# WoojuLee24/OA-DG

Measured on AMD Instinct MI355X. Metric: images/sec training, Faster R-CNN R50-FPN + OA-DG, 1024x2048, higher is better.
Workload: dtype bf16

## Files before the change

oa-dg_amd/csrc/assign.hip:

```cpp
#include <cstring>
#include "common.h"
#include "../../include/oadg_hip.h"

namespace {

constexpr int AS_THREADS = 256;
constexpr int AS_MAXG = 1024;

struct AssignArgs {
    const float* boxes;
    long box_stride;
    const unsigned char* valid;
    const float* gts;
    const int* gt_counts;
    const int64_t* gt_labels;
    int B, N, Gmax;
    float pos_thr, neg_lo, neg_hi, min_pos;
    int match_low_quality;
    unsigned* gt_max;
    int64_t* gt_inds;
    float* max_overlaps;
    int64_t* labels;
    int* counts;
    long out_stride;
};

__device__ __forceinline__ unsigned fkey(float f) {
    const unsigned u = __float_as_uint(f);
    return (u & 0x80000000u) ? ~u : (u | 0x80000000u);
}
__device__ __forceinline__ float funkey(unsigned k) {
    return __uint_as_float((k & 0x80000000u) ? (k & 0x7fffffffu) : ~k);
}

__device__ __forceinline__ float iou_of(const float4 g, const float ga, const float4 b, const float ba) {
    const float ltx = fmaxf(g.x, b.x), lty = fmaxf(g.y, b.y);
    const float rbx = fminf(g.z, b.z), rby = fminf(g.w, b.w);
    const float w = fmaxf(rbx - ltx, 0.f), h = fmaxf(rby - lty, 0.f);
    const float overlap = w * h;
    float uni = (ga + ba) - overlap;
    uni = fmaxf(uni, 1e-6f);
    return overlap / uni;
}

__global__ __launch_bounds__(AS_THREADS) void assign_gtmax_kernel(AssignArgs a) {
    __shared__ float4 sg[AS_MAXG];
    __shared__ float sga[AS_MAXG];
    __shared__ unsigned smax[AS_MAXG];
    const int b = blockIdx.y;
    const int G = a.gt_counts[b];
    for (int g = threadIdx.x; g < G; g += AS_THREADS) {
        const float4 v = reinterpret_cast<const float4*>(a.gts)[(long)b * a.Gmax + g];
        sg[g] = v;
        sga[g] = (v.z - v.x) * (v.w - v.y);
        smax[g] = fkey(-1.f);
    }
    __syncthreads();
    const float* boxes = a.boxes + (long)b * a.box_stride;
    const int lane = threadIdx.x & 63;
    const long chunk = (long)gridDim.x * AS_THREADS;
    for (long base = (long)blockIdx.x * AS_THREADS; base < a.N; base += chunk) {
        const long n = base + threadIdx.x;
        const bool ok = n < a.N && (!a.valid || a.valid[(long)b * a.N + n]);
        float4 bx = make_float4(0.f, 0.f, 0.f, 0.f);
        if (n < a.N) bx = reinterpret_cast<const float4*>(boxes)[n];
        const float ba = (bx.z - bx.x) * (bx.w - bx.y);
        for (int g = 0; g < G; ++g) {
            float v = ok ? iou_of(sg[g], sga[g], bx, ba) : -1.f;
            v = wave_max(v);
            if (lane == 0) atomicMax(&smax[g], fkey(v));
        }
    }
    __syncthreads();
    for (int g = threadIdx.x; g < G; g += AS_THREADS) atomicMax(&a.gt_max[(long)b * a.Gmax + g], smax[g]);
}

__global__ __launch_bounds__(AS_THREADS) void assign_kernel(AssignArgs a) {
    __shared__ float4 sg[AS_MAXG];
    __shared__ float sga[AS_MAXG];
    __shared__ float sgm[AS_MAXG];
    __shared__ int red[2][AS_THREADS / 64];
    const int b = blockIdx.y;
    const int G = a.gt_counts[b];
    for (int g = threadIdx.x; g < G; g += AS_THREADS) {
        const float4 v = reinterpret_cast<const float4*>(a.gts)[(long)b * a.Gmax + g];
        sg[g] = v;
        sga[g] = (v.z - v.x) * (v.w - v.y);
        sgm[g] = funkey(a.gt_max[(long)b * a.Gmax + g]);
    }
    __syncthreads();
    const float* boxes = a.boxes + (long)b * a.box_stride;
    int npos = 0, nneg = 0;
    const long chunk = (long)gridDim.x * AS_THREADS;
    for (long n = (long)blockIdx.x * AS_THREADS + threadIdx.x; n < a.N; n += chunk) {
        const bool ok = !a.valid || a.valid[(long)b * a.N + n];
        const float4 bx = reinterpret_cast<const float4*>(boxes)[n];
        const float ba = (bx.z - bx.x) * (bx.w - bx.y);
        int64_t ind = -1;
        float mo = 0.f;
        if (G == 0) {
            ind = 0;
        } else {
            float best = -2.f;
            int arg = 0, last = 0;
            for (int g = 0; g < G; ++g) {
                const float v = ok ? iou_of(sg[g], sga[g], bx, ba) : -1.f;
                if (v > best) { best = v; arg = g; }
                if (a.match_low_quality && sgm[g] >= a.min_pos && v == sgm[g]) last = g + 1;
            }
            mo = best;
            if (best >= a.neg_lo && best < a.neg_hi) ind = 0;
            if (best >= a.pos_thr) ind = arg + 1;
            if (last > 0) ind = last;
        }
        if (!ok) ind = -1;
        a.gt_inds[(long)b * a.out_stride + n] = ind;
        a.max_overlaps[(long)b * a.out_stride + n] = mo;
        if (a.labels) a.labels[(long)b * a.out_stride + n] = ind > 0 ? a.gt_labels[(long)b * a.Gmax + (ind - 1)] : -1;
        npos += ind > 0;
        nneg += ind == 0;
    }
    npos = wave_sum_i(npos);
    nneg = wave_sum_i(nneg);
    const int lane = threadIdx.x & 63, w = threadIdx.x >> 6;
    if (lane == 0) { red[0][w] = npos; red[1][w] = nneg; }
    __syncthreads();
    if (threadIdx.x == 0) {
        int p = 0, q = 0;
        for (int i = 0; i < AS_THREADS / 64; ++i) { p += red[0][i]; q += red[1][i]; }
        if (p) atomicAdd(&a.counts[b * 2], p);
        if (q) atomicAdd(&a.counts[b * 2 + 1], q);
    }
}

__global__ void assign_init_kernel(unsigned* gt_max, int n, int* counts, int m) {
    const int i = blockIdx.x * blockDim.x + threadIdx.x;
    if (i < n) gt_max[i] = fkey(-1.f);
    if (i < m) counts[i] = 0;
}

struct RoiPrepArgs {
    oadg_roi_assign_image img[OADG_ROI_ASSIGN_MAX_IMAGES];
    int B, N, Gmax;
    float* boxes_full;
    int64_t* gt_inds_full;
    int64_t* labels_full;
    float* max_ov_full;
    unsigned char* valid;
    float* gts_pad;
    int64_t* gl_pad;
    int* gt_counts;
    unsigned* gt_max;
    int* counts;
};

__global__ __launch_bounds__(256) void roi_assign_prep_kernel(const RoiPrepArgs a) {
    const int b = blockIdx.y;
    const float* props = nullptr; const float* gts = nullptr; const int64_t* gl = nullptr;
    int stride = 4, G = 0;
#pragma unroll
    for (int i = 0; i < OADG_ROI_ASSIGN_MAX_IMAGES; ++i)
        if (i == b) { props = a.img[i].proposals; gts = a.img[i].gt_bboxes; gl = a.img[i].gt_labels;
                      stride = a.img[i].stride; G = a.img[i].num_gts; }
    const int rows = a.Gmax + a.N;
    const int r = blockIdx.x * 256 + threadIdx.x;
    if (r == 0) {
        a.gt_counts[b] = G;
        a.counts[2 * b] = 0; a.counts[2 * b + 1] = 0;
        if (a.Gmax == 0) a.gt_max[b] = fkey(-1.f);
    }
    if (r >= rows) return;
    const long o = (long)b * rows + r;
    if (r < a.Gmax) {
        float4 g = make_float4(0.f, 0.f, 0.f, 0.f);
        int64_t l = 0;
        if (r < G) { g = reinterpret_cast<const float4*>(gts)[r]; l = gl[r]; }
        reinterpret_cast<float4*>(a.gts_pad)[(long)b * a.Gmax + r] = g;
        a.gl_pad[(long)b * a.Gmax + r] = l;
        a.gt_max[(long)b * a.Gmax + r] = fkey(-1.f);
        const int j = r - (a.Gmax - G);
        if (j >= 0) {
            reinterpret_cast<float4*>(a.boxes_full)[o] = reinterpret_cast<const float4*>(gts)[j];
            a.gt_inds_full[o] = j + 1;
            a.labels_full[o] = gl[j];
            a.max_ov_full[o] = 1.0f;
        }
        return;
    }
    const int n = r - a.Gmax;
    const float* p = props + (long)n * stride;
    reinterpret_cast<float4*>(a.boxes_full)[o] = make_float4(p[0], p[1], p[2], p[3]);
    a.valid[(long)b * a.N + n] = stride >= 5 ? (p[4] >= 0.f ? 1 : 0) : 1;
}

}

extern "C" size_t oadg_max_iou_assign_workspace_bytes(int B, int Gmax) {
    return B > 0 && Gmax >= 0 ? (size_t)B * (Gmax > 0 ? Gmax : 1) * sizeof(unsigned) : 0;
}

extern "C" int oadg_max_iou_assign(const float* boxes, long box_stride, const unsigned char* valid, const float* gts,
                                   const int* gt_counts, const int64_t* gt_labels, int B, int N, int Gmax,
                                   float pos_iou_thr, float neg_iou_lo, float neg_iou_hi, float min_pos_iou,
                                   int match_low_quality, void* workspace, size_t workspace_bytes, int64_t* gt_inds,
                                   float* max_overlaps, int64_t* labels, int* counts, void* stream) {
    if (!boxes || !gt_counts || !gt_inds || !max_overlaps || !counts || !workspace) return OADG_EARG;
    if (B < 1 || N < 0 || Gmax < 0 || Gmax > AS_MAXG || (Gmax > 0 && !gts) || (labels && !gt_labels)) return OADG_EARG;
    if (workspace_bytes < oadg_max_iou_assign_workspace_bytes(B, Gmax)) return OADG_ESIZE;
    AssignArgs a;
    a.boxes = boxes; a.box_stride = box_stride; a.valid = valid; a.gts = gts; a.gt_counts = gt_counts;
    a.gt_labels = gt_labels; a.B = B; a.N = N; a.Gmax = Gmax;
    a.pos_thr = pos_iou_thr; a.neg_lo = neg_iou_lo; a.neg_hi = neg_iou_hi; a.min_pos = min_pos_iou;
    a.match_low_quality = match_low_quality;
    a.gt_max = (unsigned*)workspace; a.gt_inds = gt_inds; a.max_overlaps = max_overlaps; a.labels = labels;
    a.counts = counts; a.out_stride = N;
    hipStream_t st = (hipStream_t)stream;
    const int ninit = B * (Gmax > 0 ? Gmax : 1) > 2 * B ? B * (Gmax > 0 ? Gmax : 1) : 2 * B;
    hipLaunchKernelGGL(assign_init_kernel, dim3((ninit + 255) / 256), dim3(256), 0, st, a.gt_max,
                       B * (Gmax > 0 ? Gmax : 1), counts, 2 * B);
    OADG_LAUNCH_CHECK();
    if (N == 0) return OADG_OK;
    int bx = (N + AS_THREADS - 1) / AS_THREADS;
    if (bx > 256) bx = 256;
    if (Gmax > 0) {
        hipLaunchKernelGGL(assign_gtmax_kernel, dim3(bx, B), dim3(AS_THREADS), 0, st, a);
        OADG_LAUNCH_CHECK();
    }
    hipLaunchKernelGGL(assign_kernel, dim3(bx, B), dim3(AS_THREADS), 0, st, a);
    OADG_LAUNCH_CHECK();
    return OADG_OK;
}

extern "C" int oadg_roi_assign_add_gt(const oadg_roi_assign_image* images_host, int B, int N, int Gmax, float pos_iou_thr,
                                      float neg_iou_lo, float neg_iou_hi, float min_pos_iou, int match_low_quality,
                                      float* boxes_full, int64_t* gt_inds_full, int64_t* labels_full, float* max_ov_full,
                                      unsigned char* valid, float* gts_pad, int64_t* gl_pad, int* gt_counts,
                                      void* workspace, size_t workspace_bytes, int* counts, void* stream) {
    if (!images_host || B < 1 || B > OADG_ROI_ASSIGN_MAX_IMAGES || N < 1 || Gmax < 0 || Gmax > AS_MAXG || !boxes_full ||
        !gt_inds_full || !labels_full || !max_ov_full || !valid || !gt_counts || !workspace || !counts ||
        (Gmax > 0 && (!gts_pad || !gl_pad)))
        return OADG_EARG;
    if (workspace_bytes < oadg_max_iou_assign_workspace_bytes(B, Gmax)) return OADG_ESIZE;
    RoiPrepArgs p;
    std::memset(&p, 0, sizeof(p));
    for (int i = 0; i < B; ++i) {
        const oadg_roi_assign_image& im = images_host[i];
        if (!im.proposals || im.stride < 4 || im.num_gts < 0 || im.num_gts > Gmax ||
            (im.num_gts > 0 && (!im.gt_bboxes || !im.gt_labels)))
            return OADG_EARG;
        p.img[i] = im;
    }
    p.B = B; p.N = N; p.Gmax = Gmax; p.boxes_full = boxes_full; p.gt_inds_full = gt_inds_full;
    p.labels_full = labels_full; p.max_ov_full = max_ov_full; p.valid = valid; p.gts_pad = gts_pad; p.gl_pad = gl_pad;
    p.gt_counts = gt_counts; p.gt_max = (unsigned*)workspace; p.counts = counts;
    hipStream_t st = (hipStream_t)stream;
    const int rows = Gmax + N;
    hipLaunchKernelGGL(roi_assign_prep_kernel, dim3((rows + 255) / 256, B), dim3(256), 0, st, p);
    OADG_LAUNCH_CHECK();
    AssignArgs a;
    a.boxes = boxes_full + (size_t)Gmax * 4; a.box_stride = (long)rows * 4; a.valid = valid; a.gts = gts_pad;
    a.gt_counts = gt_counts; a.gt_labels = gl_pad; a.B = B; a.N = N; a.Gmax = Gmax;
    a.pos_thr = pos_iou_thr; a.neg_lo = neg_iou_lo; a.neg_hi = neg_iou_hi; a.min_pos = min_pos_iou;
    a.match_low_quality = match_low_quality; a.gt_max = (unsigned*)workspace;
    a.gt_inds = gt_inds_full + Gmax; a.max_overlaps = max_ov_full + Gmax; a.labels = labels_full + Gmax;
    a.counts = counts; a.out_stride = rows;
    int bx = (N + AS_THREADS - 1) / AS_THREADS;
    if (bx > 256) bx = 256;
    if (Gmax > 0) {
        hipLaunchKernelGGL(assign_gtmax_kernel, dim3(bx, B), dim3(AS_THREADS), 0, st, a);
        OADG_LAUNCH_CHECK();
    }
    hipLaunchKernelGGL(assign_kernel, dim3(bx, B), dim3(AS_THREADS), 0, st, a);
    OADG_LAUNCH_CHECK();
    return OADG_OK;
}
```

oa-dg_amd/csrc/nms.hip:

```cpp
#include "common.h"
#include <type_traits>

namespace {

constexpr int MAX_WORDS_PER_LANE = 8;

__device__ __forceinline__ float iou_f32(const float4 a, const float4 b) {
    const float left = fmaxf(a.x, b.x), right = fminf(a.z, b.z);
    const float top = fmaxf(a.y, b.y), bottom = fminf(a.w, b.w);
    const float w = fmaxf(right - left, 0.f), h = fmaxf(bottom - top, 0.f);
    const float inter = w * h;
    const float sa = (a.z - a.x) * (a.w - a.y);
    const float sb = (b.z - b.x) * (b.w - b.y);
    return inter / (sa + sb - inter);
}

__global__ __launch_bounds__(64) void nms_mask_kernel(const float4* __restrict__ boxes,
                                                      const int* __restrict__ counts, int Mmax,
                                                      int words, float thr,
                                                      unsigned long long* __restrict__ mask) {
    const int img = blockIdx.z, rb = blockIdx.y, cb = blockIdx.x;
    if (cb < rb) return;
    const int M = min(counts[img], Mmax);
    if (rb * 64 >= M || cb * 64 >= M) return;
    __shared__ float4 colbox[64];
    const float4* b = boxes + (size_t)img * Mmax;
    const int t = threadIdx.x;
    const int cidx = cb * 64 + t;
    colbox[t] = cidx < M ? b[cidx] : make_float4(0.f, 0.f, 0.f, 0.f);
    __syncthreads();
    const int r = rb * 64 + t;
    if (r >= M) return;
    const float4 me = b[r];
    unsigned long long bits = 0ull;
    const int ncol = min(64, M - cb * 64);
    const int start = (rb == cb) ? t + 1 : 0;
    for (int j = start; j < ncol; ++j)
        if (iou_f32(me, colbox[j]) > thr) bits |= 1ull << j;
    mask[((size_t)img * Mmax + r) * words + cb] = bits;
}

__device__ __forceinline__ unsigned wave_or32(unsigned v) {
    v |= (unsigned)__builtin_amdgcn_update_dpp(0, (int)v, 0x128, 0xf, 0xf, false);
    v |= (unsigned)__builtin_amdgcn_update_dpp(0, (int)v, 0x124, 0xf, 0xf, false);
    v |= (unsigned)__builtin_amdgcn_update_dpp(0, (int)v, 0x122, 0xf, 0xf, false);
    v |= (unsigned)__builtin_amdgcn_update_dpp(0, (int)v, 0x121, 0xf, 0xf, false);
    return (unsigned)__builtin_amdgcn_readlane((int)v, 0) | (unsigned)__builtin_amdgcn_readlane((int)v, 16) |
           (unsigned)__builtin_amdgcn_readlane((int)v, 32) | (unsigned)__builtin_amdgcn_readlane((int)v, 48);
}
__device__ __forceinline__ unsigned long long wave_or64(unsigned long long v) {
    return ((unsigned long long)wave_or32((unsigned)(v >> 32)) << 32) | wave_or32((unsigned)v);
}

template <int SLOTS, int ROUNDS>
__global__ __launch_bounds__(64) void nms_scan_kernel(const unsigned long long* __restrict__ mask,
                                                      const int* __restrict__ counts, int Mmax,
                                                      int words, int max_keep, int* __restrict__ keep,
                                                      int* __restrict__ keep_cnt) {
    const int img = blockIdx.x, lane = threadIdx.x;
    const int M = min(counts[img], Mmax);
    const unsigned long long* mk = mask + (size_t)img * Mmax * words;
    int* out = keep + (size_t)img * Mmax;
    unsigned long long removed[SLOTS];
    unsigned long long pend[2][ROUNDS * 8][SLOTS];
#pragma unroll
    for (int s = 0; s < SLOTS; ++s) {
        removed[s] = 0ull;
#pragma unroll
        for (int u = 0; u < ROUNDS * 8; ++u) pend[0][u][s] = pend[1][u][s] = 0ull;
    }
    int nkeep = 0, pend_rounds[2] = {0, 0};
    const int nchunks = (M + 63) / 64;
    auto row_words = [&](int c, unsigned long long& d, unsigned long long& n1, unsigned long long& n2) {
        const int row = c * 64 + lane;
        const bool ok = c < nchunks && row < M;
        const unsigned long long* r = mk + (size_t)(ok ? row : 0) * words;
        d = ok ? r[c] : 0ull;
        n1 = (ok && c + 1 < nchunks) ? r[c + 1] : 0ull;
        n2 = (ok && c + 2 < nchunks) ? r[c + 2] : 0ull;
    };
    auto merge = [&](int w, unsigned long long v) {
#pragma unroll
        for (int s = 0; s < SLOTS; ++s)
            if (s == (w >> 6) && lane == (w & 63)) removed[s] |= v;
    };
    unsigned long long diag, near1, near2;
    row_words(0, diag, near1, near2);
    auto chunk = [&](int cw, auto set_c) {
        constexpr int SET = decltype(set_c)::value;
        unsigned long long mine = 0ull;
#pragma unroll
        for (int s = 0; s < SLOTS; ++s)
            if (s == (cw >> 6)) mine = removed[s];
        const unsigned lo = (unsigned)__builtin_amdgcn_readlane((int)(unsigned)mine, cw & 63);
        const unsigned hi = (unsigned)__builtin_amdgcn_readlane((int)(unsigned)(mine >> 32), cw & 63);
        unsigned long long cur = ((unsigned long long)hi << 32) | lo;
        unsigned long long ndiag, nnear1, nnear2;
        row_words(cw + 1, ndiag, nnear1, nnear2);
        const int nb = min(64, M - cw * 64);
        const int myrow = cw * 64 + lane;
        unsigned long long avail = ~cur & (nb == 64 ? ~0ull : ((1ull << nb) - 1ull));
        unsigned long long kept = 0ull;
        int nk = nkeep;
        while (avail && nk < max_keep) {
            const int bit = __ffsll((long long)avail) - 1;
            kept |= 1ull << bit;
            ++nk;
            const unsigned dlo = __builtin_amdgcn_readlane((int)(unsigned)diag, bit);
            const unsigned dhi = __builtin_amdgcn_readlane((int)(unsigned)(diag >> 32), bit);
            const unsigned long long d = ((unsigned long long)dhi << 32) | dlo;
            avail &= ~d & ~((2ull << bit) - 1ull);
        }
        const bool me_kept = (kept >> lane) & 1ull;
        if (me_kept) out[nkeep + __popcll(kept & ((1ull << lane) - 1ull))] = myrow;
        nkeep = nk;
        merge(cw + 1, wave_or64(me_kept ? near1 : 0ull));
        merge(cw + 2, wave_or64(me_kept ? near2 : 0ull));
#pragma unroll
        for (int rd = 0; rd < ROUNDS; ++rd)
            if (rd < pend_rounds[SET]) {
#pragma unroll
                for (int s = 0; s < SLOTS; ++s)
#pragma unroll
                    for (int u = 0; u < 8; ++u) removed[s] |= pend[SET][rd * 8 + u][s];
            }
        unsigned long long todo = kept;
        auto far_round = [&](int* bits) {
#pragma unroll
            for (int u = 0; u < 8; ++u) {
                bits[u] = todo ? __ffsll((long long)todo) - 1 : -1;
                todo &= todo - 1ull;
            }
        };
        pend_rounds[SET] = 0;
#pragma unroll
        for (int rd = 0; rd < ROUNDS; ++rd) {
            if (!todo) break;
            ++pend_rounds[SET];
            int bits[8];
            far_round(bits);
#pragma unroll
            for (int s = 0; s < SLOTS; ++s) {
                const int w = lane + 64 * s;
                const bool far = w > cw + 2 && w < nchunks;
#pragma unroll
                for (int u = 0; u < 8; ++u)
                    pend[SET][rd * 8 + u][s] = (far && bits[u] >= 0) ? mk[(size_t)(cw * 64 + bits[u]) * words + w] : 0ull;
            }
        }
        while (todo) {
            int bits[8];
            far_round(bits);
#pragma unroll
            for (int s = 0; s < SLOTS; ++s) {
                const int w = lane + 64 * s;
                const bool far = w > cw + 2 && w < nchunks;
                unsigned long long v[8];
#pragma unroll
                for (int u = 0; u < 8; ++u)
                    v[u] = (far && bits[u] >= 0) ? mk[(size_t)(cw * 64 + bits[u]) * words + w] : 0ull;
#pragma unroll
                for (int u = 0; u < 8; ++u) removed[s] |= v[u];
            }
        }
        diag = ndiag; near1 = nnear1; near2 = nnear2;
    };
    for (int cw = 0; cw < nchunks && nkeep < max_keep; cw += 2) {
        chunk(cw, std::integral_constant<int, 0>{});
        if (cw + 1 < nchunks && nkeep < max_keep) chunk(cw + 1, std::integral_constant<int, 1>{});
    }
    if (lane == 0) keep_cnt[img] = nkeep;
}

}

extern "C" {

size_t oadg_nms_workspace_bytes(int n_images, int Mmax) {
    if (n_images <= 0 || Mmax <= 0) return 0;
    const size_t words = (size_t)(Mmax + 63) / 64;
    return (size_t)n_images * Mmax * words * sizeof(unsigned long long);
}

int oadg_nms_batched(const float* boxes, const int* counts, int n_images, int Mmax, float iou_thr,
                     int max_keep, void* workspace, size_t workspace_bytes, int* keep, int* keep_cnt,
                     void* stream) {
    if (!boxes || !counts || !workspace || !keep || !keep_cnt) return OADG_EARG;
    if (n_images < 1 || Mmax < 1 || Mmax > 64 * 64 * MAX_WORDS_PER_LANE) return OADG_EARG;
    if (workspace_bytes < oadg_nms_workspace_bytes(n_images, Mmax)) return OADG_ESIZE;
    if (max_keep <= 0 || max_keep > Mmax) max_keep = Mmax;
    hipStream_t st = (hipStream_t)stream;
    const int words = (Mmax + 63) / 64;
    hipLaunchKernelGGL(nms_mask_kernel, dim3(words, words, n_images), dim3(64), 0, st,
                       (const float4*)boxes, counts, Mmax, words, iou_thr, (unsigned long long*)workspace);
    OADG_LAUNCH_CHECK();
    if (words <= 64 * 3)
        hipLaunchKernelGGL((nms_scan_kernel<3, 2>), dim3(n_images), dim3(64), 0, st,
                           (const unsigned long long*)workspace, counts, Mmax, words, max_keep, keep, keep_cnt);
    else
        hipLaunchKernelGGL((nms_scan_kernel<MAX_WORDS_PER_LANE, 1>), dim3(n_images), dim3(64), 0, st,
                           (const unsigned long long*)workspace, counts, Mmax, words, max_keep, keep, keep_cnt);
    OADG_LAUNCH_CHECK();
    return OADG_OK;
}

}
```

Baseline: 142.5.

## Restructure NMS into panel mask/scan passes and register-block IoU assignment

NMS now works in panels of 30 column blocks. Each panel gets a mask kernel that computes only that panel's IoU bits plus the suppression contributed by rows already kept, and a scan kernel that resolves keeps in LDS with a wave-parallel diagonal step. This avoids building and scanning the full triangular mask when max_keep stops early, but it adds per-panel launches and a more complex workspace layout. In assign, the gt-max kernel now blocks 8 GTs × 4 boxes in registers with one wave reduction per GT chunk instead of one per box-row, the assign loop is unrolled over GT chunks, and IoU skips the division when there is no overlap.

```diff
diff --git a/oa-dg_amd/csrc/assign.hip b/oa-dg_amd/csrc/assign.hip
--- a/oa-dg_amd/csrc/assign.hip
+++ b/oa-dg_amd/csrc/assign.hip
@@ -38,37 +38,59 @@
     const float rbx = fminf(g.z, b.z), rby = fminf(g.w, b.w);
     const float w = fmaxf(rbx - ltx, 0.f), h = fmaxf(rby - lty, 0.f);
     const float overlap = w * h;
+    if (!(overlap > 0.f)) return overlap;
     float uni = (ga + ba) - overlap;
     uni = fmaxf(uni, 1e-6f);
     return overlap / uni;
 }
 
+constexpr int AS_GCHUNK = 8;
+constexpr int AS_BOXES = 4;
+
 __global__ __launch_bounds__(AS_THREADS) void assign_gtmax_kernel(AssignArgs a) {
-    __shared__ float4 sg[AS_MAXG];
-    __shared__ float sga[AS_MAXG];
+    __shared__ float4 sg[AS_MAXG + AS_GCHUNK];
+    __shared__ float sga[AS_MAXG + AS_GCHUNK];
     __shared__ unsigned smax[AS_MAXG];
     const int b = blockIdx.y;
     const int G = a.gt_counts[b];
-    for (int g = threadIdx.x; g < G; g += AS_THREADS) {
-        const float4 v = reinterpret_cast<const float4*>(a.gts)[(long)b * a.Gmax + g];
+    const int Gpad = (G + AS_GCHUNK - 1) / AS_GCHUNK * AS_GCHUNK;
+    for (int g = threadIdx.x; g < Gpad; g += AS_THREADS) {
+        float4 v = make_float4(0.f, 0.f, 0.f, 0.f);
+        if (g < G) v = reinterpret_cast<const float4*>(a.gts)[(long)b * a.Gmax + g];
         sg[g] = v;
         sga[g] = (v.z - v.x) * (v.w - v.y);
-        smax[g] = fkey(-1.f);
+        if (g < G) smax[g] = fkey(-1.f);
     }
     __syncthreads();
     const float* boxes = a.boxes + (long)b * a.box_stride;
     const int lane = threadIdx.x & 63;
     const long chunk = (long)gridDim.x * AS_THREADS;
-    for (long base = (long)blockIdx.x * AS_THREADS; base < a.N; base += chunk) {
-        const long n = base + threadIdx.x;
-        const bool ok = n < a.N && (!a.valid || a.valid[(long)b * a.N + n]);
-        float4 bx = make_float4(0.f, 0.f, 0.f, 0.f);
-        if (n < a.N) bx = reinterpret_cast<const float4*>(boxes)[n];
-        const float ba = (bx.z - bx.x) * (bx.w - bx.y);
-        for (int g = 0; g < G; ++g) {
-            float v = ok ? iou_of(sg[g], sga[g], bx, ba) : -1.f;
-            v = wave_max(v);
-            if (lane == 0) atomicMax(&smax[g], fkey(v));
+    for (int g0 = 0; g0 < G; g0 += AS_GCHUNK) {
+        float4 gb[AS_GCHUNK];
+        float gar[AS_GCHUNK], m[AS_GCHUNK];
+#pragma unroll
+        for (int u = 0; u < AS_GCHUNK; ++u) { gb[u] = sg[g0 + u]; gar[u] = sga[g0 + u]; m[u] = -1.f; }
+        for (long n0 = (long)blockIdx.x * AS_THREADS + threadIdx.x; n0 < a.N; n0 += AS_BOXES * chunk) {
+            float4 bx[AS_BOXES];
+            bool ok[AS_BOXES];
+#pragma unroll
+            for (int k = 0; k < AS_BOXES; ++k) {
+                const long n = n0 + k * chunk;
+                ok[k] = n < a.N && (!a.valid || a.valid[(long)b * a.N + n]);
+                bx[k] = n < a.N ? reinterpret_cast<const float4*>(boxes)[n] : make_float4(0.f, 0.f, 0.f, 0.f);
+            }
+#pragma unroll
+            for (int k = 0; k < AS_BOXES; ++k) {
+                if (!ok[k]) continue;
+                const float ba = (bx[k].z - bx[k].x) * (bx[k].w - bx[k].y);
+#pragma unroll
+                for (int u = 0; u < AS_GCHUNK; ++u) m[u] = fmaxf(m[u], iou_of(gb[u], gar[u], bx[k], ba));
+            }
+        }
+#pragma unroll
+        for (int u = 0; u < AS_GCHUNK; ++u) {
+            const float v = wave_max(m[u]);
+            if (lane == 0 && g0 + u < G) atomicMax(&smax[g0 + u], fkey(v));
         }
     }
     __syncthreads();
@@ -103,11 +125,21 @@
         } else {
             float best = -2.f;
             int arg = 0, last = 0;
-            for (int g = 0; g < G; ++g) {
-                const float v = ok ? iou_of(sg[g], sga[g], bx, ba) : -1.f;
+            auto visit = [&](int g, const float4 gt, const float gta, const float gtm) {
+                const float v = ok ? iou_of(gt, gta, bx, ba) : -1.f;
                 if (v > best) { best = v; arg = g; }
-                if (a.match_low_quality && sgm[g] >= a.min_pos && v == sgm[g]) last = g + 1;
+                if (a.match_low_quality && gtm >= a.min_pos && v == gtm) last = g + 1;
+            };
+            int g = 0;
+            for (; g + AS_GCHUNK <= G; g += AS_GCHUNK) {
+                float4 gt[AS_GCHUNK];
+                float gta[AS_GCHUNK], gtm[AS_GCHUNK];
+#pragma unroll
+                for (int u = 0; u < AS_GCHUNK; ++u) { gt[u] = sg[g + u]; gta[u] = sga[g + u]; gtm[u] = sgm[g + u]; }
+#pragma unroll
+                for (int u = 0; u < AS_GCHUNK; ++u) visit(g + u, gt[u], gta[u], gtm[u]);
             }
+            for (; g < G; ++g) visit(g, sg[g], sga[g], sgm[g]);
             mo = best;
             if (best >= a.neg_lo && best < a.neg_hi) ind = 0;
             if (best >= a.pos_thr) ind = arg + 1;
diff --git a/oa-dg_amd/csrc/nms.hip b/oa-dg_amd/csrc/nms.hip
--- a/oa-dg_amd/csrc/nms.hip
+++ b/oa-dg_amd/csrc/nms.hip
@@ -1,44 +1,45 @@
 #include "common.h"
-#include <type_traits>
 
 namespace {
 
-constexpr int MAX_WORDS_PER_LANE = 8;
-
-__device__ __forceinline__ float iou_f32(const float4 a, const float4 b) {
+constexpr int MAX_ROWS = 64 * 64 * 8;
+constexpr int NMS_PW = 15;
+constexpr int NMS_W = 2 * NMS_PW;
+constexpr int NMS_TRI = NMS_PW * (NMS_PW + 1) / 2;
+constexpr int NMS_TRI_W = NMS_W * (NMS_W + 1) / 2;
+constexpr int NMS_LDS_STRIDE = 65;
+
+__device__ __forceinline__ bool suppresses(const float4 a, const float4 b, const float thr, const bool thr_nonneg) {
     const float left = fmaxf(a.x, b.x), right = fminf(a.z, b.z);
     const float top = fmaxf(a.y, b.y), bottom = fminf(a.w, b.w);
     const float w = fmaxf(right - left, 0.f), h = fmaxf(bottom - top, 0.f);
     const float inter = w * h;
+    if (thr_nonneg && !(inter > 0.f)) return false;
     const float sa = (a.z - a.x) * (a.w - a.y);
     const float sb = (b.z - b.x) * (b.w - b.y);
-    return inter / (sa + sb - inter);
-}
-
-__global__ __launch_bounds__(64) void nms_mask_kernel(const float4* __restrict__ boxes,
-                                                      const int* __restrict__ counts, int Mmax,
-                                                      int words, float thr,
-                                                      unsigned long long* __restrict__ mask) {
-    const int img = blockIdx.z, rb = blockIdx.y, cb = blockIdx.x;
-    if (cb < rb) return;
-    const int M = min(counts[img], Mmax);
-    if (rb * 64 >= M || cb * 64 >= M) return;
-    __shared__ float4 colbox[64];
-    const float4* b = boxes + (size_t)img * Mmax;
-    const int t = threadIdx.x;
-    const int cidx = cb * 64 + t;
-    colbox[t] = cidx < M ? b[cidx] : make_float4(0.f, 0.f, 0.f, 0.f);
-    __syncthreads();
-    const int r = rb * 64 + t;
-    if (r >= M) return;
-    const float4 me = b[r];
+    return inter / (sa + sb - inter) > thr;
+}
+
+__device__ __forceinline__ unsigned long long row_bits(const float4 me, const float4 col, float thr) {
+    const bool thr_nonneg = thr >= 0.f;
     unsigned long long bits = 0ull;
-    const int ncol = min(64, M - cb * 64);
-    const int start = (rb == cb) ? t + 1 : 0;
-    for (int j = start; j < ncol; ++j)
-        if (iou_f32(me, colbox[j]) > thr) bits |= 1ull << j;
-    mask[((size_t)img * Mmax + r) * words + cb] = bits;
-}
+#pragma unroll
+    for (int j = 0; j < 64; ++j) {
+        const float4 c = make_float4(__int_as_float(__builtin_amdgcn_readlane(__float_as_int(col.x), j)),
+                                     __int_as_float(__builtin_amdgcn_readlane(__float_as_int(col.y), j)),
+                                     __int_as_float(__builtin_amdgcn_readlane(__float_as_int(col.z), j)),
+                                     __int_as_float(__builtin_amdgcn_readlane(__float_as_int(col.w), j)));
+        if (suppresses(me, c, thr, thr_nonneg)) bits |= 1ull << j;
+    }
+    return bits;
+}
+
+__device__ __forceinline__ int tri_index(int n, int rb, int cb) { return rb * n - rb * (rb - 1) / 2 + (cb - rb); }
+
+__device__ __forceinline__ size_t word_index(bool packed, int words, int c0, int rb, int cb, int lane) {
+    return packed ? (size_t)tri_index(NMS_W, rb - c0, cb - c0) * 64 + lane : (size_t)(rb * 64 + lane) * words + cb;
+}
+constexpr size_t NMS_REMOVED_AT = (size_t)NMS_TRI_W * 64;
 
 __device__ __forceinline__ unsigned wave_or32(unsigned v) {
     v |= (unsigned)__builtin_amdgcn_update_dpp(0, (int)v, 0x128, 0xf, 0xf, false);
@@ -52,124 +53,140 @@
     return ((unsigned long long)wave_or32((unsigned)(v >> 32)) << 32) | wave_or32((unsigned)v);
 }
 
-template <int SLOTS, int ROUNDS>
-__global__ __launch_bounds__(64) void nms_scan_kernel(const unsigned long long* __restrict__ mask,
-                                                      const int* __restrict__ counts, int Mmax,
-                                                      int words, int max_keep, int* __restrict__ keep,
-                                                      int* __restrict__ keep_cnt) {
-    const int img = blockIdx.x, lane = threadIdx.x;
+__global__ __launch_bounds__(256) void nms_panel_mask_kernel(const float4* __restrict__ boxes,
+                                                            const int* __restrict__ counts, int Mmax, int words,
+                                                            float thr, int max_keep, int c0,
+                                                            const int* __restrict__ keep, const int* __restrict__ keep_cnt,
+                                                            unsigned long long* __restrict__ ws) {
+    const int img = blockIdx.z, wv = threadIdx.x >> 6, lane = threadIdx.x & 63;
     const int M = min(counts[img], Mmax);
-    const unsigned long long* mk = mask + (size_t)img * Mmax * words;
+    const int nk = c0 > 0 ? keep_cnt[img] : 0;
+    if (c0 * 64 >= M || (c0 > 0 && nk >= max_keep)) return;
+    const int kept_base = ((int)blockIdx.x - NMS_W) * 64;
+    if (kept_base >= nk) return;
+    const int c1 = min(words, c0 + NMS_W);
+    const int cb = c0 + blockIdx.y * 4 + wv;
+    const bool own = blockIdx.x < NMS_W;
+    const int rb = c0 + blockIdx.x;
+    if (cb >= c1 || cb * 64 >= M || (own && rb > cb)) return;
+    const float4* b = boxes + (size_t)img * Mmax;
+    const int cidx = cb * 64 + lane;
+    const float4 col = cidx < M ? b[cidx] : make_float4(0.f, 0.f, 0.f, 0.f);
+    const int i = own ? rb * 64 + lane : kept_base + lane;
+    const bool row_ok = i < (own ? M : nk);
+    const int r = !row_ok ? 0 : own ? i : keep[(size_t)img * Mmax + i];
+    unsigned long long bits = row_bits(b[r], col, thr);
+    const int ncol = min(64, M - cb * 64);
+    bits &= ncol == 64 ? ~0ull : (1ull << ncol) - 1ull;
+    if (own && rb == cb) bits &= ~((2ull << lane) - 1ull);
+    if (!row_ok) bits = 0ull;
+    const bool packed = words > NMS_W;
+    unsigned long long* base = ws + (size_t)img * Mmax * words;
+    if (own) {
+        if (row_ok) base[word_index(packed, words, c0, rb, cb, lane)] = bits;
+    } else {
+        bits = wave_or64(bits);
+        if (lane == 0 && bits) atomicOr(&base[NMS_REMOVED_AT + cb], bits);
+    }
+}
+
+__device__ __forceinline__ unsigned long long readlane64(unsigned long long v, int l) {
+    const unsigned lo = (unsigned)__builtin_amdgcn_readlane((int)(unsigned)v, l);
+    const unsigned hi = (unsigned)__builtin_amdgcn_readlane((int)(unsigned)(v >> 32), l);
+    return ((unsigned long long)hi << 32) | lo;
+}
+
+__global__ __launch_bounds__(1024) void nms_panel_scan_kernel(const int* __restrict__ counts, int Mmax, int words,
+                                                             int max_keep, int c0, int* __restrict__ keep,
+                                                             int* __restrict__ keep_cnt, unsigned long long* __restrict__ ws) {
+    __shared__ unsigned long long tile[NMS_TRI * NMS_LDS_STRIDE];
+    __shared__ unsigned long long kept_of[NMS_PW];
+    __shared__ unsigned long long next_removed[NMS_PW];
+    __shared__ int nkeep_shared;
+    const int img = blockIdx.x, wv = threadIdx.x >> 6, lane = threadIdx.x & 63;
+    const int M = min(counts[img], Mmax);
+    int nkeep = c0 > 0 ? keep_cnt[img] : 0;
+    if (c0 > 0 && (c0 * 64 >= M || nkeep >= max_keep)) return;
+    const int c1 = min(words, c0 + NMS_W);
+    const int nchunks = (M + 63) / 64;
+    const bool packed = words > NMS_W;
+    unsigned long long* base = ws + (size_t)img * Mmax * words;
     int* out = keep + (size_t)img * Mmax;
-    unsigned long long removed[SLOTS];
-    unsigned long long pend[2][ROUNDS * 8][SLOTS];
-#pragma unroll
-    for (int s = 0; s < SLOTS; ++s) {
-        removed[s] = 0ull;
-#pragma unroll
-        for (int u = 0; u < ROUNDS * 8; ++u) pend[0][u][s] = pend[1][u][s] = 0ull;
-    }
-    int nkeep = 0, pend_rounds[2] = {0, 0};
-    const int nchunks = (M + 63) / 64;
-    auto row_words = [&](int c, unsigned long long& d, unsigned long long& n1, unsigned long long& n2) {
-        const int row = c * 64 + lane;
-        const bool ok = c < nchunks && row < M;
-        const unsigned long long* r = mk + (size_t)(ok ? row : 0) * words;
-        d = ok ? r[c] : 0ull;
-        n1 = (ok && c + 1 < nchunks) ? r[c + 1] : 0ull;
-        n2 = (ok && c + 2 < nchunks) ? r[c + 2] : 0ull;
-    };
-    auto merge = [&](int w, unsigned long long v) {
-#pragma unroll
-        for (int s = 0; s < SLOTS; ++s)
-            if (s == (w >> 6) && lane == (w & 63)) removed[s] |= v;
-    };
-    unsigned long long diag, near1, near2;
-    row_words(0, diag, near1, near2);
-    auto chunk = [&](int cw, auto set_c) {
-        constexpr int SET = decltype(set_c)::value;
-        unsigned long long mine = 0ull;
-#pragma unroll
-        for (int s = 0; s < SLOTS; ++s)
-            if (s == (cw >> 6)) mine = removed[s];
-        const unsigned lo = (unsigned)__builtin_amdgcn_readlane((int)(unsigned)mine, cw & 63);
-        const unsigned hi = (unsigned)__builtin_amdgcn_readlane((int)(unsigned)(mine >> 32), cw & 63);
-        unsigned long long cur = ((unsigned long long)hi << 32) | lo;
-        unsigned long long ndiag, nnear1, nnear2;
-        row_words(cw + 1, ndiag, nnear1, nnear2);
-        const int nb = min(64, M - cw * 64);
-        const int myrow = cw * 64 + lane;
-        unsigned long long avail = ~cur & (nb == 64 ? ~0ull : ((1ull << nb) - 1ull));
-        unsigned long long kept = 0ull;
-        int nk = nkeep;
-        while (avail && nk < max_keep) {
-            const int bit = __ffsll((long long)avail) - 1;
-            kept |= 1ull << bit;
-            ++nk;
-            const unsigned dlo = __builtin_amdgcn_readlane((int)(unsigned)diag, bit);
-            const unsigned dhi = __builtin_amdgcn_readlane((int)(unsigned)(diag >> 32), bit);
-            const unsigned long long d = ((unsigned long long)dhi << 32) | dlo;
-            avail &= ~d & ~((2ull << bit) - 1ull);
-        }
-        const bool me_kept = (kept >> lane) & 1ull;
-        if (me_kept) out[nkeep + __popcll(kept & ((1ull << lane) - 1ull))] = myrow;
-        nkeep = nk;
-        merge(cw + 1, wave_or64(me_kept ? near1 : 0ull));
-        merge(cw + 2, wave_or64(me_kept ? near2 : 0ull));
-#pragma unroll
-        for (int rd = 0; rd < ROUNDS; ++rd)
-            if (rd < pend_rounds[SET]) {
-#pragma unroll
-                for (int s = 0; s < SLOTS; ++s)
-#pragma unroll
-                    for (int u = 0; u < 8; ++u) removed[s] |= pend[SET][rd * 8 + u][s];
+    const int t = lane & 15, q = lane >> 4;
+    for (int h0 = c0; h0 < c1; h0 += NMS_PW) {
+        if (h0 > c0) {
+            nkeep = nkeep_shared;
+            if (h0 * 64 >= M || nkeep >= max_keep) break;
+        }
+        const int h1 = min(c1, h0 + NMS_PW);
+        const int nch = min(h1, nchunks) - h0;
+        unsigned long long v[8];
+#pragma unroll
+        for (int u = 0; u < 8; ++u) {
+            const int blk = wv + 16 * u;
+            int rb = 0, off = blk;
+            while (off >= NMS_PW - rb && rb < NMS_PW - 1) { off -= NMS_PW - rb; ++rb; }
+            const int cb = rb + off;
+            v[u] = 0ull;
+            if (blk < NMS_TRI && cb < nch && (h0 + rb) * 64 + lane < M)
+                v[u] = base[word_index(packed, words, c0, h0 + rb, h0 + cb, lane)];
+        }
+#pragma unroll
+        for (int u = 0; u < 8; ++u)
+            if (wv + 16 * u < NMS_TRI) tile[(wv + 16 * u) * NMS_LDS_STRIDE + lane] = v[u];
+        unsigned long long removed = 0ull;
+        if (wv == 0 && lane < nch) {
+            if (c0 > 0) removed = base[NMS_REMOVED_AT + h0 + lane];
+            if (h0 > c0) removed |= next_removed[lane];
+        }
+        __syncthreads();
+        if (wv == 0) {
+            if (lane < NMS_PW) { kept_of[lane] = 0ull; next_removed[lane] = 0ull; }
+            for (int c = 0; c < nch && nkeep < max_keep; ++c) {
+                const unsigned long long cur = readlane64(removed, c) | readlane64(removed, c + 16) |
+                                               readlane64(removed, c + 32) | readlane64(removed, c + 48);
+                const unsigned long long diag = tile[tri_index(NMS_PW, c, c) * NMS_LDS_STRIDE + lane];
+                const int nb = min(64, M - (h0 + c) * 64);
+                unsigned long long undecided = ~cur & (nb == 64 ? ~0ull : ((1ull << nb) - 1ull));
+                unsigned long long kept = 0ull;
+                while (undecided) {
+                    const unsigned long long hit = wave_or64(((undecided >> lane) & 1ull) ? diag : 0ull);
+                    const unsigned long long safe = undecided & ~hit;
+                    kept |= safe;
+                    undecided &= ~safe & ~wave_or64(((safe >> lane) & 1ull) ? diag : 0ull);
+                }
+                for (int over = nkeep + __popcll(kept) - max_keep; over > 0; --over)
+                    kept &= ~(1ull << (63 - __clzll((long long)kept)));
+                if ((kept >> lane) & 1ull) out[nkeep + __popcll(kept & ((1ull << lane) - 1ull))] = (h0 + c) * 64 + lane;
+                nkeep += __popcll(kept);
+                if (lane == 0) kept_of[c] = kept;
+                if (t > c && t < nch) {
+                    const unsigned long long* blk = tile + tri_index(NMS_PW, c, t) * NMS_LDS_STRIDE + 16 * q;
+                    const unsigned mine = (unsigned)(kept >> (16 * q)) & 0xffffu;
+#pragma unroll
+                    for (int r = 0; r < 16; ++r) removed |= blk[r] & (0ull - (unsigned long long)((mine >> r) & 1u));
+                }
             }
-        unsigned long long todo = kept;
-        auto far_round = [&](int* bits) {
-#pragma unroll
-            for (int u = 0; u < 8; ++u) {
-                bits[u] = todo ? __ffsll((long long)todo) - 1 : -1;
-                todo &= todo - 1ull;
+            if (lane == 0) nkeep_shared = nkeep;
+        }
+        __syncthreads();
+        const int n2 = min(c1, nchunks) - h1;
+        if (h0 == c0 && n2 > 0 && nkeep_shared < max_keep && wv < nch) {
+            const bool mine = (kept_of[wv] >> lane) & 1ull;
+            unsigned long long w2[NMS_PW];
+#pragma unroll
+            for (int j = 0; j < NMS_PW; ++j)
+                w2[j] = (mine && j < n2) ? base[word_index(packed, words, c0, h0 + wv, h1 + j, lane)] : 0ull;
+#pragma unroll
+            for (int j = 0; j < NMS_PW; ++j) {
+                const unsigned long long o = wave_or64(w2[j]);
+                if (lane == 0 && o) atomicOr(&next_removed[j], o);
             }
-        };
-        pend_rounds[SET] = 0;
-#pragma unroll
-        for (int rd = 0; rd < ROUNDS; ++rd) {
-            if (!todo) break;
-            ++pend_rounds[SET];
-            int bits[8];
-            far_round(bits);
-#pragma unroll
-            for (int s = 0; s < SLOTS; ++s) {
-                const int w = lane + 64 * s;
-                const bool far = w > cw + 2 && w < nchunks;
-#pragma unroll
-                for (int u = 0; u < 8; ++u)
-                    pend[SET][rd * 8 + u][s] = (far && bits[u] >= 0) ? mk[(size_t)(cw * 64 + bits[u]) * words + w] : 0ull;
-            }
-        }
-        while (todo) {
-            int bits[8];
-            far_round(bits);
-#pragma unroll
-            for (int s = 0; s < SLOTS; ++s) {
-                const int w = lane + 64 * s;
-                const bool far = w > cw + 2 && w < nchunks;
-                unsigned long long v[8];
-#pragma unroll
-                for (int u = 0; u < 8; ++u)
-                    v[u] = (far && bits[u] >= 0) ? mk[(size_t)(cw * 64 + bits[u]) * words + w] : 0ull;
-#pragma unroll
-                for (int u = 0; u < 8; ++u) removed[s] |= v[u];
-            }
-        }
-        diag = ndiag; near1 = nnear1; near2 = nnear2;
-    };
-    for (int cw = 0; cw < nchunks && nkeep < max_keep; cw += 2) {
-        chunk(cw, std::integral_constant<int, 0>{});
-        if (cw + 1 < nchunks && nkeep < max_keep) chunk(cw + 1, std::integral_constant<int, 1>{});
-    }
-    if (lane == 0) keep_cnt[img] = nkeep;
+        }
+        __syncthreads();
+    }
+    if (threadIdx.x == 0) keep_cnt[img] = nkeep;
+    if (packed && threadIdx.x < NMS_W && c1 + (int)threadIdx.x < words) base[NMS_REMOVED_AT + c1 + threadIdx.x] = 0ull;
 }
 
 }
@@ -186,21 +203,21 @@
                      int max_keep, void* workspace, size_t workspace_bytes, int* keep, int* keep_cnt,
                      void* stream) {
     if (!boxes || !counts || !workspace || !keep || !keep_cnt) return OADG_EARG;
-    if (n_images < 1 || Mmax < 1 || Mmax > 64 * 64 * MAX_WORDS_PER_LANE) return OADG_EARG;
+    if (n_images < 1 || Mmax < 1 || Mmax > MAX_ROWS) return OADG_EARG;
     if (workspace_bytes < oadg_nms_workspace_bytes(n_images, Mmax)) return OADG_ESIZE;
     if (max_keep <= 0 || max_keep > Mmax) max_keep = Mmax;
     hipStream_t st = (hipStream_t)stream;
     const int words = (Mmax + 63) / 64;
-    hipLaunchKernelGGL(nms_mask_kernel, dim3(words, words, n_images), dim3(64), 0, st,
-                       (const float4*)boxes, counts, Mmax, words, iou_thr, (unsigned long long*)workspace);
-    OADG_LAUNCH_CHECK();
-    if (words <= 64 * 3)
-        hipLaunchKernelGGL((nms_scan_kernel<3, 2>), dim3(n_images), dim3(64), 0, st,
-                           (const unsigned long long*)workspace, counts, Mmax, words, max_keep, keep, keep_cnt);
-    else
-        hipLaunchKernelGGL((nms_scan_kernel<MAX_WORDS_PER_LANE, 1>), dim3(n_images), dim3(64), 0, st,
-                           (const unsigned long long*)workspace, counts, Mmax, words, max_keep, keep, keep_cnt);
-    OADG_LAUNCH_CHECK();
+    for (int c0 = 0; c0 < words; c0 += NMS_W) {
+        const int kept_groups = ((max_keep < c0 * 64 ? max_keep : c0 * 64) + 63) / 64;
+        hipLaunchKernelGGL(nms_panel_mask_kernel, dim3(NMS_W + kept_groups, (NMS_W + 3) / 4, n_images), dim3(256), 0, st,
+                           (const float4*)boxes, counts, Mmax, words, iou_thr, max_keep, c0, (const int*)keep,
+                           (const int*)keep_cnt, (unsigned long long*)workspace);
+        OADG_LAUNCH_CHECK();
+        hipLaunchKernelGGL(nms_panel_scan_kernel, dim3(n_images), dim3(1024), 0, st, counts, Mmax, words, max_keep, c0,
+                           keep, keep_cnt, (unsigned long long*)workspace);
+        OADG_LAUNCH_CHECK();
+    }
     return OADG_OK;
 }
 
```

After: 144.0 (median of 6 runs). About the same (+1.1%).
